# neptune-ai/open-solution-salt-identification

Measured on AMD Instinct MI355X. Metric: training images/sec, U-Net ResNet34 101x101 (pad->128) bs32/GPU, higher is better.
Workload: dtype bf16; 1 GPU; architectures.unet.UNetResNet(34, hypercolumn) 128x128 (101 resized+edge-padded) batch 32/GPU, lovasz loss, Adam lr1e-4 L2 1e-4, train-mode BN; global_batch=32, parallelism=dp1

## Files before the change

include/saltnet.h:

```cpp
#ifndef SALTNET_H
#define SALTNET_H
#include <stdint.h>

#ifdef __cplusplus
extern "C" {
#endif

#define SALT_F32 0
#define SALT_BF16 1

#define SALT_OK 0
#define SALT_E_BADARG -1
#define SALT_E_UNSUPPORTED -2
#define SALT_E_LDS -3

#define SALT_MAX_TAPS 16

typedef struct {
    void* p;
    int B;
    int H;
    int W;
    int C;
    int cs;
// ... 183 lines not shown

typedef struct {
    int dtype;
    const float* w;
    int Cout;
    int Cin;
    int K;
    void* wp;
} salt_pack_stem_weight_args;
int salt_pack_stem_weight(const salt_pack_stem_weight_args*, void* stream);

typedef struct {
    const float* g16;
    int Cout;
    int Cin;
    int K;
    float* grad;
    int accumulate;
} salt_stem_grad_unfold_args;
int salt_stem_grad_unfold(const salt_stem_grad_unfold_args*, void* stream);

typedef struct {
    int dtype;
    salt_view x;
    const float* w;
    const float* bias;
    int Cout;
    float* y_nchw;
    salt_view y;
} salt_head1x1_args;
int salt_head1x1(const salt_head1x1_args*, void* stream);
int salt_head1x1_kernel_id(const salt_head1x1_args*);

typedef struct {
    int dtype;
    salt_view x;
    const float* w;
    int Cout;
    const float* dy_nchw;
    salt_view dx;
    int accumulate;
    float* partials;
    int nparts;
    float* gw;
    float* gb;
} salt_head1x1_bwd_args;
// ... 361 lines not shown
    const float* grad;
    float* exp_avg;
    float* exp_avg_sq;
    int64_t n;
    const float* hyper;
} salt_adam_args;
int salt_adam(const salt_adam_args*, void* stream);

typedef struct {
    float* param;
    const float* grad;
    float* exp_avg;
    float* exp_avg_sq;
    int64_t n;
    const float* hyper;
    const void* jobs;
    const int* job_block0;
    int njobs;
    int pack_blocks;
    const int64_t* rest;
    const int* rest_block0;
    int nrest;
    int rest_blocks;
} salt_adam_pack_args;
int salt_adam_pack(const salt_adam_pack_args*, void* stream);
int salt_pack_job_is_vec(const salt_pack_conv_weight_args*);

typedef struct {
    float* hyper;
    int64_t* step;
} salt_adam_tick_args;
int salt_adam_tick(const salt_adam_tick_args*, void* stream);

typedef struct {
    void* p;
    int64_t bytes;
} salt_zero_args;
int salt_zero(const salt_zero_args*, void* stream);

typedef struct {
    const float* logits;
    int V;
    int B;
    int C;
    int H;
    int W;
// ... 412 lines not shown
```

open-solution-salt-identification_amd/csrc/build.py:

```python
import hashlib
import os
import subprocess
import sys
from concurrent.futures import ThreadPoolExecutor

HERE = os.path.dirname(os.path.abspath(__file__))
PKG = os.path.dirname(HERE)
ROOT = os.path.dirname(PKG)
INC = os.path.join(ROOT, 'include')
OBJ = os.path.join(HERE, '_obj')
LIB = os.path.join(PKG, 'libsaltnet_hip.so')
SOURCES = ['runtime.hip', 'conv_mfma.hip', 'conv_wgrad.hip', 'conv_ws.hip', 'conv_thin.hip', 'conv_wgrad_ls.hip', 'conv_small.hip', 'head_fused.hip', 'elementwise.hip', 'hyper.hip', 'se.hip', 'se_res.hip', 'conv_group.hip', 'dense.hip', 'depth.hip', 'classifier.hip', 'stacking.hip', 'loss.hip', 'input.hip', 'augment.hip']
FLAGS = ['--offload-arch=gfx950', '-O3', '-std=c++17', '-fPIC', '-I' + INC, '-I' + HERE, '-Wno-unused-value']


def _hipcc():
    for c in (os.environ.get('HIPCC'), '/opt/rocm/bin/hipcc', 'hipcc'):
        if c and (os.path.isabs(c) and os.path.exists(c) or not os.path.isabs(c)):
            return c
    raise RuntimeError('hipcc not found')


def _digest(path):
    h = hashlib.sha1()
    for p in [path, os.path.join(HERE, 'common.h'), os.path.join(HERE, 'preprocess_common.h'), os.path.join(INC, 'saltnet.h')]:
        with open(p, 'rb') as f:
            h.update(f.read())
    h.update(' '.join(FLAGS).encode())
    return h.hexdigest()


def _compile(src):
    path = os.path.join(HERE, src)
    obj = os.path.join(OBJ, src.replace('.hip', '.o'))
    stamp = obj + '.sha1'
# ... 35 lines not shown
```

open-solution-salt-identification_amd/csrc/conv_mfma.hip:

```cpp
#include <cstdlib>
#include <type_traits>
#include "common.h"

namespace {

struct ConvKP {
    const void* x; const void* w; void* y;
    const float* bias; const float* scale; const float* shift;
    float* stats; float* stats_cnt;
    int B, H, W, Cin, x_cs;
    int Cout, y_cs, OHf, OWf, OH, OW, out_step, out_oy, out_ox;
    int ntaps; int tap_off[SALT_MAX_TAPS];
    int in_step, pad_mode, min_dy, min_dx;
    int th_log2, tw_log2, nb;
    int gen, tw, th, twth;
    unsigned tw_magic, twth_magic;
    int hh, hw;
    int tiles_y, tiles_x;
    int nchunk, a_bytes;
    int relu, accumulate, stats_part0;
    void* strip; int strip_cs, fold_top, fold_bottom, fold_left, fold_right;
    int nphase, m_tiles_ph; int64_t w_phase_elems;
    int fold_fused, ox_shift;
    unsigned hhw_magic, hw_magic;
// ... 1598 lines not shown
        return;
    }
    for (int e = threadIdx.x; e < PACK_EPB; e += 256) {
        const int64_t i = base + e;
        if (i >= total) break;
        const int kc = (int)(i % KCE);
        int64_t r = i / KCE;
        const int n = (int)(r % N); r /= N;
        const int t = (int)(r % a.ntaps);
        const int ch = (int)(r / a.ntaps) * KCE + kc;
        float v = 0.f;
        if (ch < C && a.tap_kh[t] >= 0) {
            const int d0 = a.transpose ? ch : n, d1 = a.transpose ? n : ch;
            v = a.w[(((int64_t)d0 * a.D1 + d1) * a.KH + a.tap_kh[t]) * a.KW + a.tap_kw[t]];
        }
        Elem<T>::st(out + ((((int64_t)(r / a.ntaps) + a.chunk_off) * a.ntaps + t) * NT_ + n + a.n_off) * KCE + kc, v);
    }
}

struct AdamPackKP {
    float* p; const float* g; float* m; float* v; const float* hyper;
    const salt_pack_conv_weight_args* jobs; const int* job_block0; int njobs, pack_blocks;
    const int64_t* rest; const int* rest_block0; int nrest;
};
constexpr int AP_SEG = 64, AP_SEGF = 288;
__global__ __launch_bounds__(256) void adam_pack_kernel(AdamPackKP k) {
    extern __shared__ __attribute__((aligned(16))) float ap_sm[];
    const float lr = k.hyper[0], b1 = k.hyper[1], b2 = k.hyper[2], eps = k.hyper[3], wd = k.hyper[4], bc1 = k.hyper[5], bc2 = k.hyper[6], gs = k.hyper[7];
    const float step_size = lr / bc1, rs = 1.f / sqrtf(bc2);
    const int tid = threadIdx.x;
    if ((int)blockIdx.x < k.pack_blocks) {
        int lo = 0, hi = k.njobs - 1;
        while (lo < hi) { const int mid = (lo + hi + 1) >> 1; if (k.job_block0[mid] <= (int)blockIdx.x) lo = mid; else hi = mid - 1; }
        const salt_pack_conv_weight_args& a = k.jobs[lo];
        const int N = a.D0, C = a.D1, nseg = N * (C / 32);
        const int seg0 = ((int)blockIdx.x - k.job_block0[lo]) * AP_SEG;
        const int64_t wbase = a.w - k.p;
#pragma unroll 3
        for (int it = 0; it < AP_SEG * AP_SEGF / 4 / 256; ++it) {
            const int f = tid + 256 * it, sl = f / (AP_SEGF / 4), fi = f - sl * (AP_SEGF / 4), seg = seg0 + sl;
            if (seg < nseg) {
                const int chunk = seg / N, n = seg - chunk * N;
                const int64_t off = wbase + ((int64_t)n * C + chunk * 32) * 9 + 4 * fi;
                f32x4 pp = *reinterpret_cast<const f32x4*>(k.p + off);
                const f32x4 gg = *reinterpret_cast<const f32x4*>(k.g + off);
                f32x4 mm = *reinterpret_cast<const f32x4*>(k.m + off), vv = *reinterpret_cast<const f32x4*>(k.v + off);
                adam4(pp, gg, mm, vv, b1, b2, eps, wd, gs, step_size, rs);
                *reinterpret_cast<f32x4*>(k.p + off) = pp; *reinterpret_cast<f32x4*>(k.m + off) = mm; *reinterpret_cast<f32x4*>(k.v + off) = vv;
                *reinterpret_cast<f32x4*>(ap_sm + sl * AP_SEGF + 4 * fi) = pp;
            }
        }
        __syncthreads();
        const int sl = tid >> 2, q = tid & 3, seg = seg0 + sl;
        if (seg >= nseg) return;
        const int chunk = seg / N, n = seg - chunk * N;
        const float* v = ap_sm + sl * AP_SEGF + q * 72;
        bf16_t* out = reinterpret_cast<bf16_t*>(a.wp);
#pragma unroll
        for (int t = 0; t < 9; ++t) {
            u32x4 o;
            o.x = f2bf_pk(v[0 * 9 + t], v[1 * 9 + t]); o.y = f2bf_pk(v[2 * 9 + t], v[3 * 9 + t]);
            o.z = f2bf_pk(v[4 * 9 + t], v[5 * 9 + t]); o.w = f2bf_pk(v[6 * 9 + t], v[7 * 9 + t]);
            *reinterpret_cast<u32x4*>(out + (((int64_t)chunk * 9 + t) * N + n) * 32 + q * 8) = o;
        }
        return;
    }
    const int rb = (int)blockIdx.x - k.pack_blocks;
    int lo = 0, hi = k.nrest - 1;
    while (lo < hi) { const int mid = (lo + hi + 1) >> 1; if (k.rest_block0[mid] <= rb) lo = mid; else hi = mid - 1; }
    const int64_t first = k.rest[2 * lo], count = k.rest[2 * lo + 1];
    const int64_t e = (int64_t)(rb - k.rest_block0[lo]) * 1024 + tid * 4;
    if (e >= count) return;
    const int64_t off = first + e;
    f32x4 pp = *reinterpret_cast<const f32x4*>(k.p + off);
    const f32x4 gg = *reinterpret_cast<const f32x4*>(k.g + off);
    f32x4 mm = *reinterpret_cast<const f32x4*>(k.m + off), vv = *reinterpret_cast<const f32x4*>(k.v + off);
    adam4(pp, gg, mm, vv, b1, b2, eps, wd, gs, step_size, rs);
    *reinterpret_cast<f32x4*>(k.p + off) = pp; *reinterpret_cast<f32x4*>(k.m + off) = mm; *reinterpret_cast<f32x4*>(k.v + off) = vv;
}

}

extern "C" int salt_conv(const salt_conv_args* a, void* stream) {
    Plan pl;
    int rc = make_plan(a, &pl);
    if (rc) return rc;
// ... 75 lines not shown
    if (pack_vec_ok(*a, a->dtype)) return (int)(((int64_t)N * (C / 32) * 4 + 255) / 256);
    if (!a->transpose) return (int)(((int64_t)N * cdiv(C, KCE) * KCE + 255) / 256);
    const int64_t total = (int64_t)cdiv(C, KCE) * a->ntaps * N * KCE;
    return (int)((total + PACK_EPB - 1) / PACK_EPB);
}

extern "C" int salt_pack_job_is_vec(const salt_pack_conv_weight_args* a) {
    return a && !a->transpose && a->KH * a->KW == 9 && pack_vec_ok(*a, a->dtype) ? 1 : 0;
}

extern "C" int salt_adam_pack(const salt_adam_pack_args* a, void* stream) {
    if (!a || !a->param || !a->grad || !a->exp_avg || !a->exp_avg_sq || !a->hyper || a->n < 0 || a->njobs < 0 || a->nrest < 0 || a->pack_blocks < 0 ||
        a->rest_blocks < 0 || (a->njobs && (!a->jobs || !a->job_block0)) || (a->nrest && (!a->rest || !a->rest_block0)))
        SALT_FAIL(SALT_E_BADARG, "adam_pack: bad args");
    if ((reinterpret_cast<uintptr_t>(a->param) | reinterpret_cast<uintptr_t>(a->grad) | reinterpret_cast<uintptr_t>(a->exp_avg) | reinterpret_cast<uintptr_t>(a->exp_avg_sq)) & 15)
        SALT_FAIL(SALT_E_BADARG, "adam_pack: buffers must be 16-byte aligned");
    const int64_t blocks = (int64_t)a->pack_blocks + a->rest_blocks;
    if (blocks == 0) return SALT_OK;
    if (blocks >= (1LL << 31)) SALT_FAIL(SALT_E_UNSUPPORTED, "adam_pack: too many blocks");
    AdamPackKP k;
    k.p = a->param; k.g = a->grad; k.m = a->exp_avg; k.v = a->exp_avg_sq; k.hyper = a->hyper;
    k.jobs = reinterpret_cast<const salt_pack_conv_weight_args*>(a->jobs); k.job_block0 = a->job_block0; k.njobs = a->njobs; k.pack_blocks = a->pack_blocks;
    k.rest = a->rest; k.rest_block0 = a->rest_block0; k.nrest = a->nrest;
    return salt_launch(adam_pack_kernel, dim3((unsigned)blocks), dim3(256), AP_SEG * AP_SEGF * sizeof(float), (hipStream_t)stream, k);
}

extern "C" int salt_pack_batched(const salt_pack_batched_args* a, void* stream) {
    if (!a || !a->jobs || !a->job_block0 || a->njobs < 1 || a->total_blocks < 1) SALT_FAIL(SALT_E_BADARG, "pack_batched: bad args");
    const auto* jobs = reinterpret_cast<const salt_pack_conv_weight_args*>(a->jobs);
    if (a->dtype == SALT_F32) hipLaunchKernelGGL(pack_batched_kernel<float>, dim3(a->total_blocks), dim3(256), 0, (hipStream_t)stream, jobs, a->job_block0, a->njobs);
    else if (a->dtype == SALT_BF16) hipLaunchKernelGGL(pack_batched_kernel<bf16_t>, dim3(a->total_blocks), dim3(256), 0, (hipStream_t)stream, jobs, a->job_block0, a->njobs);
    else SALT_FAIL(SALT_E_BADARG, "pack_batched: dtype");
    SALT_CHECK_LAUNCH();
    return SALT_OK;
}
```

open-solution-salt-identification_amd/csrc/runtime.hip:

```cpp
#include <stdarg.h>
#include <string.h>
#include <stdlib.h>
#include "common.h"

static thread_local char g_err[512] = "";

void salt_set_error(const char* fmt, ...) {
    va_list ap;
    va_start(ap, fmt);
    vsnprintf(g_err, sizeof(g_err), fmt, ap);
    va_end(ap);
}

extern "C" const char* salt_last_error(void) { return g_err; }

extern "C" int salt_abi_version(void) { return 30; }

extern "C" int salt_device_info(int* cu_count, int* lds_bytes, char* arch_name, int arch_name_len) {
    int dev = 0;
    hipError_t e = hipGetDevice(&dev);
    if (e != hipSuccess) SALT_FAIL((int)e, "hipGetDevice: %s", hipGetErrorString(e));
    hipDeviceProp_t prop;
    e = hipGetDeviceProperties(&prop, dev);
    if (e != hipSuccess) SALT_FAIL((int)e, "hipGetDeviceProperties: %s", hipGetErrorString(e));
    if (cu_count) *cu_count = prop.multiProcessorCount;
    if (lds_bytes) *lds_bytes = (int)prop.sharedMemPerBlock;
    if (arch_name && arch_name_len > 0) { strncpy(arch_name, prop.gcnArchName, arch_name_len - 1); arch_name[arch_name_len - 1] = 0; }
    return SALT_OK;
}

extern "C" int salt_program_run_range(const salt_program_entry* e, int begin, int end, void* stream) {
    if (!e || begin < 0 || end < begin) SALT_FAIL(SALT_E_BADARG, "program: bad range");
    for (int i = begin; i < end; ++i) {
        const int rc = e[i].fn(e[i].args, stream);
        if (rc) {
            char prev[400];
            strncpy(prev, g_err, sizeof(prev) - 1); prev[sizeof(prev) - 1] = 0;
            salt_set_error("program entry %d failed (%d): %s", i, rc, prev);
            return rc;
// ... 210 lines not shown
extern "C" int salt_zero(const salt_zero_args* a, void* stream) {
    if (!a || !a->p || a->bytes < 0 || (a->bytes & 3)) SALT_FAIL(SALT_E_BADARG, "zero: bad args");
    if (a->bytes == 0) return SALT_OK;
    const int64_t n4 = a->bytes / 4;
    const int blocks = (int)((n4 + 255) / 256 < 2048 ? (n4 + 255) / 256 : 2048);
    hipLaunchKernelGGL(zero_kernel, dim3(blocks), dim3(256), 0, (hipStream_t)stream, (uint32_t*)a->p, n4);
    SALT_CHECK_LAUNCH();
    return SALT_OK;
}

extern "C" int salt_abi_struct_sizes(int* out, int n) {
    static const int sizes[] = {
    (int)sizeof(salt_view),
    (int)sizeof(salt_conv_args),
    (int)sizeof(salt_conv_wgrad_args),
    (int)sizeof(salt_wgrad_reduce_args),
    (int)sizeof(salt_pack_conv_weight_args),
    (int)sizeof(salt_pack_batched_args),
    (int)sizeof(salt_conv_first_args),
    (int)sizeof(salt_conv_first_wgrad_args),
    (int)sizeof(salt_s2d_args),
    (int)sizeof(salt_pack_stem_weight_args),
    (int)sizeof(salt_stem_grad_unfold_args),
    (int)sizeof(salt_head1x1_args),
    (int)sizeof(salt_head1x1_bwd_args),
    (int)sizeof(salt_bn_finalize_args),
    (int)sizeof(salt_bn_fold_args),
    (int)sizeof(salt_affine_act_args),
    (int)sizeof(salt_bn_bwd_args),
    (int)sizeof(salt_head_bn_args),
    (int)sizeof(salt_head_bn_bwd_args),
    (int)sizeof(salt_relu_bwd_args),
    (int)sizeof(salt_maxpool2_args),
    (int)sizeof(salt_maxpool2_bwd_args),
    (int)sizeof(salt_avgpool2_args),
    (int)sizeof(salt_bilinear_args),
    (int)sizeof(salt_hyper_stencil_args),
    (int)sizeof(salt_pad_fold_args),
    (int)sizeof(salt_pad_fold_strip_args),
    (int)sizeof(salt_add_args),
    (int)sizeof(salt_layout_args),
    (int)sizeof(salt_scse_args),
    (int)sizeof(salt_scse_bwd_args),
    (int)sizeof(salt_depth_gate_args),
    (int)sizeof(salt_channel_gate_args),
    (int)sizeof(salt_lovasz_args),
// ... 32 lines not shown
```

open-solution-salt-identification_amd/engine.py:

```python
import contextlib
import ctypes
from collections import namedtuple
from dataclasses import dataclass, field
from typing import Any

import numpy as np
import torch

from . import switches
from ._abi import OP_FUNCS, STRUCTS, SaltError, check, fill, lib

DT_CODE = {'f32': 0, 'bf16': 1}
TORCH_DT = {'f32': torch.float32, 'bf16': torch.bfloat16}
VEC = {'f32': 4, 'bf16': 8}

PARTIALS_OWN = 0
PARTIALS_FILLED = 1
PARTIALS_FINALIZED = 2
PARTIALS_SHARDS = 3

SUMS_OWN = 'own'
SUMS_CONV = 'conv'
SUMS_SEC = 'sec'
SUMS_SCSE = 'scse'
# ... 1059 lines not shown
            self.tape.append(backward)
        else:
            w = eng.bn_work(bn)
            self.fwd.add('conv_first', y=out.view(), scale=w['scale'].data_ptr(), shift=w['shift'].data_ptr(), relu=int(relu), **common)
        return out

    def _stem_s2d(self, x_nchw, conv, bn, relu, name):
        eng = self.engine
        B, Cin, H, W = x_nchw.shape
        Cout, _, K, _ = conv.weight.shape
        TT, half = (K + 1) // 2, (K + 1) // 4
        z = self.new_act(B, H // 2, W // 2, 16, name + '.s2d')
        self.fwd.add('s2d', dtype=self.dt, x=x_nchw.data_ptr(), B=B, Cin=Cin, H=H, W=W, z=z.view())
        wp = eng.packed_stem(conv)
        taps = [(dh - half, dw - half) for dh in range(TT) for dw in range(TT)]
        OH, OW = H // 2, W // 2
        out = self.new_act(B, OH, OW, Cout, name)
        if self.train:
            y = self.new_act(B, OH, OW, Cout, name + '.y')
            w, _ = self._conv_bn_train(z, y, [(wp.data_ptr(), taps, 1, 0, OH, OW, {})], bn, relu, None, out, self._scratch_sfx)

            def backward():
                self._bn_train_bwd(y, bn, relu, None, out, w)
                g16 = self.f32(Cout * 16 * TT * TT)
                gw_tmp = g16.data_ptr()
                per = 8 if len(taps) > 9 else 9
                for i in range(0, len(taps), per):
                    chunk = list(range(i, min(i + per, len(taps))))
                    wg = dict(dtype=self.dt, ntaps=len(chunk), tap_dy=[taps[j][0] for j in chunk], tap_dx=[taps[j][1] for j in chunk], q_step=1, pad_mode=0)
                    ns = lib.salt_conv_wgrad_nsplit(ctypes.byref(fill(STRUCTS['salt_conv_wgrad_args'](), p=y.gview(), q=z.view(), **wg)))
                    nbytes = ns * len(chunk) * Cout * 16 * 4
                    self.bwd.add('conv_wgrad', stream=0, p=y.gview(), q=z.view(), partials=Scratch('wgrad@main', nbytes), nsplit=ns, **wg)
                    self.bwd.add('wgrad_reduce', stream=0, partials=Scratch('wgrad@main', nbytes), nsplit=ns, ntaps=len(chunk), Ca=Cout, Cb=16, KH=TT, KW=TT,
                                 tap_kh=[j // TT for j in chunk], tap_kw=[j % TT for j in chunk], grad=gw_tmp, accumulate=0)
                self.bwd.add('stem_grad_unfold', stream=0, g16=gw_tmp, Cout=Cout, Cin=Cin, K=K, grad=self._gp(conv.weight), accumulate=0)
            self.tape.append(backward)
        else:
            w = eng.bn_work(bn)
            self._conv_launch(self.fwd, z.view(), wp.data_ptr(), taps, 1, 0, out.view(), OH, OW,
                              scale=w['scale'].data_ptr(), shift=w['shift'].data_ptr(), relu=int(relu))
        return out

    def stack_conv(self, x_nchw, conv, bn, relu=True, head=None, gate=None, logits=None, name='stack'):
        eng = self.engine
        B, M, H, W = x_nchw.shape
        F = conv.weight.shape[0]
# ... 474 lines not shown
```

open-solution-salt-identification_amd/optim.py:

```python

import torch

from ._abi import SaltError
from .engine import Program


def weight_regularization(model, regularize, weight_decay_conv2d):
    params = [p for p in model.parameters() if p.requires_grad]
    if regularize:
        return [{'params': params, 'weight_decay': weight_decay_conv2d}]
    return [params]


class FusedAdam(torch.optim.Optimizer):

    def __init__(self, param_groups, lr=1e-3, betas=(0.9, 0.999), eps=1e-8, weight_decay=0.0, model=None):
        if isinstance(param_groups, (list, tuple)) and param_groups and isinstance(param_groups[0], dict):
            g = dict(param_groups[0])
        else:
            g = {'params': list(param_groups[0] if param_groups and isinstance(param_groups[0], (list, tuple)) else param_groups)}
        super().__init__([g], dict(lr=lr, betas=betas, eps=eps, weight_decay=weight_decay))
        if len(self.param_groups) != 1:
            raise SaltError('FusedAdam: one parameter group (models.py:289-297)')
        self.param_groups[0].setdefault('initial_lr', self.param_groups[0]['lr'])
# ... 5 lines not shown

    def _bind(self):
        eng = self.model.engine()
        if self._eng is eng:
            return
        old = (self.exp_avg, self.exp_avg_sq) if self._eng is not None else None
        self._eng = eng
        dev = eng.device
        if old is not None and old[0].numel() == eng.flat.numel():
            self.exp_avg, self.exp_avg_sq = old[0].to(dev).clone(), old[1].to(dev).clone()
        else:
            if old is not None:
                self.steps = 0
            self.exp_avg = torch.zeros_like(eng.flat)
            self.exp_avg_sq = torch.zeros_like(eng.flat)
        self.hyper = torch.zeros(8, dtype=torch.float32, device=dev)
        self.step_t = torch.full((1,), self.steps, dtype=torch.int64, device=dev)
        self._host_hyper = None
        self.prog = Program('adam')
        self.prog.add('adam_tick', hyper=self.hyper.data_ptr(), step=self.step_t.data_ptr())
        self.prog.add('adam', param=eng.flat.data_ptr(), grad=eng.grads.data_ptr(), exp_avg=self.exp_avg.data_ptr(),
                      exp_avg_sq=self.exp_avg_sq.data_ptr(), n=eng.n_live, hyper=self.hyper.data_ptr())
        self.prog.finalize()
        self._pack_prog, self._pack_gen = None, None

    def _adam_pack_program(self):
        import numpy as np
        eng = self._eng
        if eng.dtype != 'bf16':
            return None
        if eng._pack_batched_n != len(eng._pack_ops):
            eng._build_pack_batch()
            eng._packed_version = eng._packed_bwd_version = -1
        if self._pack_gen == eng._pack_generation:
            return self._pack_prog
        self._pack_gen, self._pack_prog = eng._pack_generation, None
        jobs = eng._adam_jobs
        if not jobs:
            return None
        import ctypes
        from ._abi import lib
        base = eng.flat.data_ptr()
        blocks = [lib.salt_pack_job_blocks(ctypes.byref(j)) for j in jobs]
        pref = np.concatenate([[0], np.cumsum(blocks)]).astype(np.int32)
        covered = sorted(((j.w - base) // 4, j.D0 * j.D1 * j.KH * j.KW) for j in jobs)
        rest, pos = [], 0
        for first, cnt in covered:
            if first % 4 or cnt % 4 or first < pos:
                return None
            if first > pos:
                rest.append((pos, first - pos))
            pos = first + cnt
        if pos < eng.n_live:
            rest.append((pos, eng.n_live - pos))
        rblocks = [(c + 1023) // 1024 for _, c in rest]
        rpref = np.concatenate([[0], np.cumsum(rblocks)]).astype(np.int32) if rest else np.zeros(1, np.int32)
        dev = eng.device
        self._pack_tables = [torch.frombuffer(bytearray(b''.join(bytes(j) for j in jobs)), dtype=torch.uint8).to(dev), torch.from_numpy(pref).to(dev),
                             torch.tensor(rest if rest else [[0, 0]], dtype=torch.int64).to(dev), torch.from_numpy(rpref).to(dev)]
        t = self._pack_tables
        prog = Program('adam_pack')
        prog.add('adam_tick', hyper=self.hyper.data_ptr(), step=self.step_t.data_ptr())
        prog.add('adam_pack', param=eng.flat.data_ptr(), grad=eng.grads.data_ptr(), exp_avg=self.exp_avg.data_ptr(), exp_avg_sq=self.exp_avg_sq.data_ptr(),
                 n=eng.n_live, hyper=self.hyper.data_ptr(), jobs=t[0].data_ptr(), job_block0=t[1].data_ptr(), njobs=len(jobs), pack_blocks=int(pref[-1]),
                 rest=t[2].data_ptr(), rest_block0=t[3].data_ptr(), nrest=len(rest), rest_blocks=int(rpref[-1]))
        prog.finalize()
        self._pack_prog = prog
        return prog

    def _sync_hyper(self):
        g = self.param_groups[0]
        cur = (float(g['lr']), float(g['betas'][0]), float(g['betas'][1]), float(g['eps']), float(g['weight_decay']), float(self.grad_scale))
        if cur != self._host_hyper:
            self.hyper[:5].copy_(torch.tensor(cur[:5], dtype=torch.float32))
            self.hyper[7:8].fill_(cur[5])
            self._host_hyper = cur

    def zero_grad(self, set_to_none=False):
        pass

    def step(self, closure=None):
        if self.model is None:
            raise SaltError('FusedAdam needs the HipNetwork it optimises (model=...)')
        self._bind()
        fused = self._adam_pack_program()
        self._sync_hyper()
        (fused or self.prog).run()
        self.steps += 1
        self._eng.touch(weights=True, stats=False)
        if fused is not None:
            self._eng._adam_packed_version = self._eng.wver

    def state_dict(self):
        g = {k: v for k, v in self.param_groups[0].items() if k != 'params'}
        g['params'] = list(range(len(self.param_groups[0]['params'])))
        st = {}
        if self._eng is None and self.model is not None and getattr(self.model, '_engine', None) is not None:
            self._bind()
        if self._eng is not None:
            st = {'step': self.steps, 'exp_avg': self.exp_avg.detach().cpu(), 'exp_avg_sq': self.exp_avg_sq.detach().cpu()}
        return {'state': st, 'param_groups': [g]}

    def load_state_dict(self, sd):
        for k, v in sd['param_groups'][0].items():
            if k != 'params':
                self.param_groups[0][k] = v
        st = sd.get('state', {})
        if st:
            self._bind()
            self.steps = int(st['step'])
            self.step_t.fill_(self.steps)
            self.exp_avg.copy_(st['exp_avg'])
            self.exp_avg_sq.copy_(st['exp_avg_sq'])
```

open-solution-salt-identification_amd/runtime.py:

```python
import ctypes

import torch

from . import _abi
from ._abi import SaltError, lib
from .engine import Graph, Program, DT_CODE, TORCH_DT


def _require_gpu(device):
    if device.type != 'cuda':
        raise SaltError('the HIP path needs a GPU tensor/device (got %s); there is no CPU fallback' % device)


def _ptr_fields(struct, ptr, out):
    for name, ct in struct._fields_:
        v = getattr(struct, name)
        if isinstance(v, ctypes.Structure):
            _ptr_fields(v, ptr, out)
        elif isinstance(v, ctypes.Array):
            for e in v:
                if isinstance(e, ctypes.Structure):
                    _ptr_fields(e, ptr, out)
        elif ct is ctypes.c_void_p and v == ptr:
            out.append((struct, name))
# ... 103 lines not shown
class Engine:
    def __init__(self, module, device, dtype='f32'):
        _require_gpu(device)
        if dtype not in DT_CODE:
            raise SaltError('dtype must be f32 or bf16')
        self.module, self.device, self.dtype = module, device, dtype
        self._flatten()
        self._packed = {}
        self._pack_ops = Program('pack')
        self._packed_bwd_version = -1
        self._pack_is_bwd, self._pack_keys = {}, []
        self._bn = {}
        self._fold_ops = Program('bn_fold')
        self.nets = {}
        self.wver = 0
        self.sver = 0
        self._packed_version = -1
        self._folded_version = None
        self.world = 1
        self.side_stream = torch.cuda.Stream(device=device)
        self._pack_generation = 0
        self._pack_batched_n = -1
        self._adam_packed_version = None
        self._graph_stream = None
        self._pack_fork = None
        self.eager_done = set()

    def _flatten(self):
        m = self.module
        dead = set(m.dead_parameter_names()) if hasattr(m, 'dead_parameter_names') else set()
        seen = {}
        live = []
        for name, p in m.named_parameters():
            if id(p) in seen:
                continue
            seen[id(p)] = name
            if p.requires_grad and name not in dead:
                live.append((name, p))
        total = sum(((p.numel() + 3) // 4) * 4 for _, p in live)
        self.flat = torch.zeros(total, dtype=torch.float32, device=self.device)
        self.grads = torch.zeros(total, dtype=torch.float32, device=self.device)
        self._off = {}
        self.live_names = []
        off = 0
        for name, p in live:
            n = p.numel()
# ... 140 lines not shown
                pref = np.concatenate([[0], np.cumsum(blocks)]).astype(np.int32)
                table = torch.frombuffer(bytearray(raw), dtype=torch.uint8).to(self.device)
                pref_t = torch.from_numpy(pref).to(self.device)
                self._pack_tables += [table, pref_t]
                prog.add('pack_batched', jobs=table.data_ptr(), job_block0=pref_t.data_ptr(), njobs=len(sel), total_blocks=int(pref[-1]),
                         dtype=DT_CODE[self.dtype])
            return prog
        fwd_jobs = [s for s, k in zip(jobs, self._pack_keys) if not self._pack_is_bwd[k]]
        fwd = batch(fwd_jobs, 'pack')
        fwd.extend(others)
        fwd.finalize()
        lo, hi = self.flat.data_ptr(), self.flat.data_ptr() + 4 * self.n_live
        seen, self._adam_jobs = set(), []
        for s in fwd_jobs:
            if lib.salt_pack_job_is_vec(ctypes.byref(s)) and lo <= s.w < hi and s.w not in seen:
                seen.add(s.w)
                self._adam_jobs.append(s)
        ids = {id(s) for s in self._adam_jobs}
        rest = batch([s for s in fwd_jobs if id(s) not in ids], 'pack_rest')
        rest.extend(others)
        rest.finalize()
        self._pack_batched_rest = rest
        self._adam_packed_version = None
        bwd = batch([s for s, k in zip(jobs, self._pack_keys) if self._pack_is_bwd[k]], 'pack_bwd')
        bwd.finalize()
        self._pack_batched, self._pack_batched_bwd = fwd, bwd
        self._pack_batched_n = len(self._pack_ops)
        self._pack_generation += 1

    def refresh(self, train):
        if self._pack_batched_n != len(self._pack_ops):
            self._build_pack_batch()
            self._packed_version = self._packed_bwd_version = -1
        if self._packed_version != self.wver:
            (self._pack_batched_rest if self._adam_packed_version == self.wver else self._pack_batched).run()
            self._packed_version = self.wver
        if train and self._packed_bwd_version != self.wver and len(self._pack_batched_bwd):
            self.side_stream.wait_stream(torch.cuda.current_stream())
            self._pack_batched_bwd.run(stream=self.side_stream)
            self._packed_bwd_version = self.wver
        if not train and self._folded_version != (self.wver, self.sver):
            self._fold_ops.run()
            self._folded_version = (self.wver, self.sver)

    def net(self, shape, train):
        key = (tuple(shape), bool(train))
        if key not in self.nets:
            self.nets[key] = CompiledNet(self, tuple(shape), train, self.module.num_classes)
        return self.nets[key]

    def step_graph(self, net, kind, loss_scale, optimizer):
        cache = net.__dict__.setdefault('_step_graphs', {})
        key = (kind, float(loss_scale))
        if self._pack_batched_n != len(self._pack_ops):
            self._build_pack_batch()
        hit = cache.get(key)
        if hit is not None and hit[0] is optimizer and hit[2] == self._pack_generation:
            return hit[1]
        if hit is not None:
            lib.salt_graph_destroy(hit[1])
        optimizer._bind()
        optimizer._sync_hyper()
# ... 69 lines not shown
```

open-solution-salt-identification_amd/switches.py:

```python
import os


def _nonempty(raw):
    return bool(raw)


def _not0(raw):
    return raw != '0'


def _on(raw):
    return raw not in ('', '0')


SWITCHES = {
    'SALT_LIB': ('', str, 'path of a libsaltnet_hip.so build variant to load instead of the package\'s own (tools/build_variant.sh)'),
    'SALT_DTYPE': ('f32', str, 'compute dtype of a network that does not name one (f32 | bf16)'),
    'SALT_STEP_GRAPH': (None, lambda raw: bool(int(raw)), '1 / 0: replay the one-GPU training step as a hipGraph; unset: training_config[\'step_graph\']'),
    'SALT_BN_FIN': (2, int, 'how train-mode BatchNorm sums travel: 2 fp64 shard atomics finalized by the consumer, 1 finalized in the producing launch, 0 per-tile partials (fixed summation order)'),
    'SALT_SE_SHARDS': (True, _not0, '0: scSE per-image sums through per-part partials (fixed summation order) instead of the fp64 shards'),
    'SALT_FWD_BN_FOLD': (False, _on, '1: BatchNorm apply + ReLU folded into the consuming convolution\'s loader; such a graph is forward-only'),
    'SALT_NO_PLANAR': (False, _nonempty, 'hypercolumn stored as channel-interleaved rows instead of dense planes'),
    'SALT_NO_SHORTCUT_FIRST': (False, _nonempty, 'projection shortcut emitted after the main branch, as the reference orders it'),
    'SALT_NO_RES_FOLD': (False, _nonempty, 'residual add + ReLU as separate launches instead of the BatchNorm apply\'s epilogue'),
    'SALT_BNB_SEC': (True, _not0, '0: a projection shortcut\'s BatchNorm backward keeps its own reduction pass'),
    'SALT_HEAD_BN': (True, _not0, '0: final BatchNorm apply and 1x1 logit head as separate launches'),
    'SALT_HYPER_FACTOR': (4, int, 'hypercolumn levels up-sampled by at least this factor enter the final convolution factored (0: none)'),
    'SALT_SE_IN_BN': (True, _not0, '0: scSE reads a materialised activation instead of applying BatchNorm + ReLU itself'),
    'SALT_SE_FC_SIDE': (True, _not0, '0: scSE backward\'s FC weight gradients on the main stream'),
    'SALT_SE_BNB': (True, _not0, '0: scSE backward does not carry the BatchNorm-backward sums of its input\'s producer'),
    'SALT_SE_RES_IN_BN': (True, _not0, '0: the SE-ResNet block tail reads the materialised BatchNorm output instead of applying scale / shift itself (measured 0.2 ms per step slower, DESIGN 16; tools/seresnet_bench.py)'),
    'SALT_RCCL_MAX_NCHANNELS': (0, int, '> 0: export NCCL_MAX_NCHANNELS=<n> before the process group is created'),
    'SALT_NO_PIN': (False, _nonempty, 'leave the process\'s CPU affinity alone'),
    'SALT_FORCE_DP_PATH': (False, _nonempty, 'one rank runs the bucketed all-reduce backward (bench.py, tools/dp_overhead.py)'),
}


def get(name):
    try:
        default, parse, _ = SWITCHES[name]
    except KeyError:
        raise KeyError('%s is not a switch of this package (switches.SWITCHES)' % name) from None
    raw = os.environ.get(name)
    return default if raw is None else parse(raw)
```

Measured before the change: 6475 images/s.

## Add dedicated stem weight-gradient kernel and emit transposed backward weights from Adam pack

```diff
diff --git a/include/saltnet.h b/include/saltnet.h
--- a/include/saltnet.h
+++ b/include/saltnet.h
@@ -229,6 +229,25 @@
 
 typedef struct {
     int dtype;
+    salt_view p;
+    salt_view q;
+    float* partials;
+    int nsplit;
+} salt_stem_wgrad_args;
+int salt_stem_wgrad_nsplit(const salt_stem_wgrad_args*);
+int salt_stem_wgrad(const salt_stem_wgrad_args*, void* stream);
+
+typedef struct {
+    const float* partials;
+    int nsplit;
+    int Cin;
+    float* grad;
+    int accumulate;
+} salt_stem_wgrad_reduce_args;
+int salt_stem_wgrad_reduce(const salt_stem_wgrad_reduce_args*, void* stream);
+
+typedef struct {
+    int dtype;
     salt_view x;
     const float* w;
     const float* bias;
@@ -636,6 +655,7 @@
     const int* rest_block0;
     int nrest;
     int rest_blocks;
+    const void* wp_t;
 } salt_adam_pack_args;
 int salt_adam_pack(const salt_adam_pack_args*, void* stream);
 int salt_pack_job_is_vec(const salt_pack_conv_weight_args*);
diff --git a/open-solution-salt-identification_amd/csrc/build.py b/open-solution-salt-identification_amd/csrc/build.py
--- a/open-solution-salt-identification_amd/csrc/build.py
+++ b/open-solution-salt-identification_amd/csrc/build.py
@@ -10,7 +10,7 @@
 INC = os.path.join(ROOT, 'include')
 OBJ = os.path.join(HERE, '_obj')
 LIB = os.path.join(PKG, 'libsaltnet_hip.so')
-SOURCES = ['runtime.hip', 'conv_mfma.hip', 'conv_wgrad.hip', 'conv_ws.hip', 'conv_thin.hip', 'conv_wgrad_ls.hip', 'conv_small.hip', 'head_fused.hip', 'elementwise.hip', 'hyper.hip', 'se.hip', 'se_res.hip', 'conv_group.hip', 'dense.hip', 'depth.hip', 'classifier.hip', 'stacking.hip', 'loss.hip', 'input.hip', 'augment.hip']
+SOURCES = ['runtime.hip', 'conv_mfma.hip', 'conv_wgrad.hip', 'conv_ws.hip', 'conv_thin.hip', 'conv_wgrad_ls.hip', 'conv_small.hip', 'stem_wgrad.hip', 'head_fused.hip', 'elementwise.hip', 'hyper.hip', 'se.hip', 'se_res.hip', 'conv_group.hip', 'dense.hip', 'depth.hip', 'classifier.hip', 'stacking.hip', 'loss.hip', 'input.hip', 'augment.hip']
 FLAGS = ['--offload-arch=gfx950', '-O3', '-std=c++17', '-fPIC', '-I' + INC, '-I' + HERE, '-Wno-unused-value']
 
 
diff --git a/open-solution-salt-identification_amd/csrc/conv_mfma.hip b/open-solution-salt-identification_amd/csrc/conv_mfma.hip
--- a/open-solution-salt-identification_amd/csrc/conv_mfma.hip
+++ b/open-solution-salt-identification_amd/csrc/conv_mfma.hip
@@ -1644,6 +1644,7 @@
     float* p; const float* g; float* m; float* v; const float* hyper;
     const salt_pack_conv_weight_args* jobs; const int* job_block0; int njobs, pack_blocks;
     const int64_t* rest; const int* rest_block0; int nrest;
+    void* const* wp_t;
 };
 constexpr int AP_SEG = 64, AP_SEGF = 288;
 __global__ __launch_bounds__(256) void adam_pack_kernel(AdamPackKP k) {
@@ -1674,16 +1675,31 @@
         }
         __syncthreads();
         const int sl = tid >> 2, q = tid & 3, seg = seg0 + sl;
-        if (seg >= nseg) return;
-        const int chunk = seg / N, n = seg - chunk * N;
-        const float* v = ap_sm + sl * AP_SEGF + q * 72;
-        bf16_t* out = reinterpret_cast<bf16_t*>(a.wp);
-#pragma unroll
-        for (int t = 0; t < 9; ++t) {
+        if (seg < nseg) {
+            const int chunk = seg / N, n = seg - chunk * N;
+            const float* v = ap_sm + sl * AP_SEGF + q * 72;
+            bf16_t* out = reinterpret_cast<bf16_t*>(a.wp);
+#pragma unroll
+            for (int t = 0; t < 9; ++t) {
+                u32x4 o;
+                o.x = f2bf_pk(v[0 * 9 + t], v[1 * 9 + t]); o.y = f2bf_pk(v[2 * 9 + t], v[3 * 9 + t]);
+                o.z = f2bf_pk(v[4 * 9 + t], v[5 * 9 + t]); o.w = f2bf_pk(v[6 * 9 + t], v[7 * 9 + t]);
+                *reinterpret_cast<u32x4*>(out + (((int64_t)chunk * 9 + t) * N + n) * 32 + q * 8) = o;
+            }
+        }
+        bf16_t* out_t = k.wp_t ? reinterpret_cast<bf16_t*>(k.wp_t[lo]) : nullptr;
+        if (!out_t) return;
+#pragma unroll
+        for (int it = 0; it < 9; ++it) {
+            const int pi = tid + 256 * it, h = pi / 1152, r = pi - h * 1152;
+            const int t = r >> 7, ci = (r >> 2) & 31, qt = r & 3, segh = seg0 + 32 * h;
+            if (segh >= nseg) continue;
+            const int chunk = segh / N, n0 = segh - chunk * N;
+            const float* v = ap_sm + (32 * h + qt * 8) * AP_SEGF + ci * 9 + t;
             u32x4 o;
-            o.x = f2bf_pk(v[0 * 9 + t], v[1 * 9 + t]); o.y = f2bf_pk(v[2 * 9 + t], v[3 * 9 + t]);
-            o.z = f2bf_pk(v[4 * 9 + t], v[5 * 9 + t]); o.w = f2bf_pk(v[6 * 9 + t], v[7 * 9 + t]);
-            *reinterpret_cast<u32x4*>(out + (((int64_t)chunk * 9 + t) * N + n) * 32 + q * 8) = o;
+            o.x = f2bf_pk(v[0], v[AP_SEGF]); o.y = f2bf_pk(v[2 * AP_SEGF], v[3 * AP_SEGF]);
+            o.z = f2bf_pk(v[4 * AP_SEGF], v[5 * AP_SEGF]); o.w = f2bf_pk(v[6 * AP_SEGF], v[7 * AP_SEGF]);
+            *reinterpret_cast<u32x4*>(out_t + (((int64_t)(n0 >> 5) * 9 + t) * C + chunk * 32 + ci) * 32 + qt * 8) = o;
         }
         return;
     }
@@ -1805,6 +1821,7 @@
     k.p = a->param; k.g = a->grad; k.m = a->exp_avg; k.v = a->exp_avg_sq; k.hyper = a->hyper;
     k.jobs = reinterpret_cast<const salt_pack_conv_weight_args*>(a->jobs); k.job_block0 = a->job_block0; k.njobs = a->njobs; k.pack_blocks = a->pack_blocks;
     k.rest = a->rest; k.rest_block0 = a->rest_block0; k.nrest = a->nrest;
+    k.wp_t = reinterpret_cast<void* const*>(a->wp_t);
     return salt_launch(adam_pack_kernel, dim3((unsigned)blocks), dim3(256), AP_SEG * AP_SEGF * sizeof(float), (hipStream_t)stream, k);
 }
 
diff --git a/open-solution-salt-identification_amd/csrc/runtime.hip b/open-solution-salt-identification_amd/csrc/runtime.hip
--- a/open-solution-salt-identification_amd/csrc/runtime.hip
+++ b/open-solution-salt-identification_amd/csrc/runtime.hip
@@ -14,7 +14,7 @@
 
 extern "C" const char* salt_last_error(void) { return g_err; }
 
-extern "C" int salt_abi_version(void) { return 30; }
+extern "C" int salt_abi_version(void) { return 31; }
 
 extern "C" int salt_device_info(int* cu_count, int* lds_bytes, char* arch_name, int arch_name_len) {
     int dev = 0;
@@ -271,6 +271,8 @@
     (int)sizeof(salt_s2d_args),
     (int)sizeof(salt_pack_stem_weight_args),
     (int)sizeof(salt_stem_grad_unfold_args),
+    (int)sizeof(salt_stem_wgrad_args),
+    (int)sizeof(salt_stem_wgrad_reduce_args),
     (int)sizeof(salt_head1x1_args),
     (int)sizeof(salt_head1x1_bwd_args),
     (int)sizeof(salt_bn_finalize_args),
diff --git a/open-solution-salt-identification_amd/csrc/stem_wgrad.hip b/open-solution-salt-identification_amd/csrc/stem_wgrad.hip
--- /dev/null
+++ b/open-solution-salt-identification_amd/csrc/stem_wgrad.hip
@@ -0,0 +1,165 @@
+#include "common.h"
+
+namespace {
+
+constexpr int SW_TW = 16, SW_TH = 8, SW_PIX = SW_TW * SW_TH;
+constexpr int SW_HW = SW_TW + 3, SW_HH = SW_TH + 3;
+constexpr int SW_PROWB = 192, SW_QROWB = 32;
+constexpr int SW_NP = SW_PIX * 8 / 256;
+constexpr int SW_QPIECES = SW_HW * SW_HH * 2, SW_NQ = (SW_QPIECES + 255) / 256;
+constexpr int SW_SLAB = 64 * 256;
+constexpr int SW_MAX_SPLIT = 256;
+constexpr int SW_RG = 16;
+
+struct StemWgradKP {
+    const bf16_t* P; const bf16_t* Q; float* partials;
+    int B, OH, OW, p_cs, q_cs;
+    int tiles_y, tiles_x, ntiles, nsplit;
+};
+
+__global__ __launch_bounds__(256) void stem_wgrad_kernel(StemWgradKP p) {
+    typedef short s16x4 __attribute__((ext_vector_type(4)));
+    typedef short s16x8 __attribute__((ext_vector_type(8)));
+    typedef __attribute__((address_space(3))) s16x4* lds_s16x4_ptr;
+    __shared__ __attribute__((aligned(16))) unsigned char sP[SW_PIX * SW_PROWB];
+    __shared__ __attribute__((aligned(16))) unsigned char sQ[SW_HW * SW_HH * SW_QROWB];
+    const int tid = threadIdx.x, lane = tid & 63, wave = tid >> 6;
+    const int split = blockIdx.x;
+
+    f32x16 acc[2][2];
+#pragma unroll
+    for (int i = 0; i < 4; ++i)
+#pragma unroll
+        for (int r = 0; r < 16; ++r) acc[i >> 1][i & 1][r] = 0.f;
+
+    int p_ty[SW_NP], p_tx[SW_NP], q_hy[SW_NQ], q_hx[SW_NQ];
+#pragma unroll
+    for (int k = 0; k < SW_NP; ++k) { const int m = (tid + (k << 8)) >> 3; p_ty[k] = m >> 4; p_tx[k] = m & 15; }
+#pragma unroll
+    for (int k = 0; k < SW_NQ; ++k) { const int hp = (tid + (k << 8)) >> 1; q_hy[k] = hp / SW_HW; q_hx[k] = hp - q_hy[k] * SW_HW; }
+    const int p_ch = (tid & 7) * 8, q_ch = (tid & 1) * 8;
+    u32x4 rp[SW_NP], rq[SW_NQ];
+    auto load_tile = [&](int tile) {
+        const int txi = tile % p.tiles_x, tt = tile / p.tiles_x, tyi = tt % p.tiles_y, b = tt / p.tiles_y;
+        const int y0 = tyi * SW_TH, x0 = txi * SW_TW;
+        const bf16_t* Pb = p.P + (int64_t)b * p.OH * p.OW * p.p_cs;
+        const bf16_t* Qb = p.Q + (int64_t)b * p.OH * p.OW * p.q_cs;
+#pragma unroll
+        for (int k = 0; k < SW_NP; ++k) {
+            const int oy = y0 + p_ty[k], ox = x0 + p_tx[k];
+            rp[k] = u32x4{0u, 0u, 0u, 0u};
+            if (oy < p.OH && ox < p.OW) rp[k] = *reinterpret_cast<const u32x4*>(Pb + (oy * p.OW + ox) * p.p_cs + p_ch);
+        }
+#pragma unroll
+        for (int k = 0; k < SW_NQ; ++k) {
+            const int iy = y0 + q_hy[k] - 2, ix = x0 + q_hx[k] - 2;
+            rq[k] = u32x4{0u, 0u, 0u, 0u};
+            if (tid + (k << 8) < SW_QPIECES && (unsigned)iy < (unsigned)p.OH && (unsigned)ix < (unsigned)p.OW)
+                rq[k] = *reinterpret_cast<const u32x4*>(Qb + (iy * p.OW + ix) * p.q_cs + q_ch);
+        }
+    };
+
+    const int khalf = lane >> 5, g16 = (lane >> 4) & 1, i16 = lane & 15, prow = i16 >> 2, pcol = (i16 & 3) * 4;
+    const int pa_base = (khalf * 8 + prow) * SW_PROWB + (g16 * 16 + pcol) * 2;
+    const int qa_base = (wave * SW_HW + khalf * 8 + prow + g16) * SW_QROWB + pcol * 2;
+
+    if (split < p.ntiles) load_tile(split);
+    for (int tile = split; tile < p.ntiles; tile += p.nsplit) {
+        __syncthreads();
+#pragma unroll
+        for (int k = 0; k < SW_NP; ++k) { const int q = tid + (k << 8); *reinterpret_cast<u32x4*>(sP + (q >> 3) * SW_PROWB + (q & 7) * 16) = rp[k]; }
+#pragma unroll
+        for (int k = 0; k < SW_NQ; ++k) { const int q = tid + (k << 8); if (q < SW_QPIECES) *reinterpret_cast<u32x4*>(sQ + q * 16) = rq[k]; }
+        __syncthreads();
+        if (tile + p.nsplit < p.ntiles) load_tile(tile + p.nsplit);
+#pragma unroll
+        for (int j = 0; j < SW_TH; ++j) {
+            s16x4 fa[2][2], fb[2][2];
+#pragma unroll
+            for (int i = 0; i < 2; ++i)
+#pragma unroll
+                for (int h = 0; h < 2; ++h) {
+                    fa[i][h] = __builtin_amdgcn_ds_read_tr16_b64_v4i16((lds_s16x4_ptr)(sP + pa_base + (j * SW_TW + 4 * h) * SW_PROWB + i * 64));
+                    fb[i][h] = __builtin_amdgcn_ds_read_tr16_b64_v4i16((lds_s16x4_ptr)(sQ + qa_base + (j * SW_HW + 4 * h + 2 * i) * SW_QROWB));
+                }
+#pragma unroll
+            for (int at = 0; at < 2; ++at) {
+                const s16x8 av = {fa[at][0][0], fa[at][0][1], fa[at][0][2], fa[at][0][3], fa[at][1][0], fa[at][1][1], fa[at][1][2], fa[at][1][3]};
+#pragma unroll
+                for (int nt = 0; nt < 2; ++nt) {
+                    const s16x8 bv = {fb[nt][0][0], fb[nt][0][1], fb[nt][0][2], fb[nt][0][3], fb[nt][1][0], fb[nt][1][1], fb[nt][1][2], fb[nt][1][3]};
+                    acc[at][nt] = __builtin_amdgcn_mfma_f32_32x32x16_bf16(__builtin_bit_cast(bf16x8, bv), __builtin_bit_cast(bf16x8, av), acc[at][nt], 0, 0, 0);
+                }
+            }
+        }
+    }
+    float* slab = p.partials + (int64_t)split * SW_SLAB;
+#pragma unroll
+    for (int at = 0; at < 2; ++at)
+#pragma unroll
+        for (int nt = 0; nt < 2; ++nt)
+#pragma unroll
+            for (int g = 0; g < 4; ++g) {
+                const int a = at * 32 + (lane & 31);
+                const int n = (wave * 4 + nt * 2) * 16 + 8 * g + 4 * khalf;
+                const f32x16& v = acc[at][nt];
+                *reinterpret_cast<f32x4*>(slab + ((n >> 2) * 64 + a) * 4) = f32x4{v[4 * g], v[4 * g + 1], v[4 * g + 2], v[4 * g + 3]};
+            }
+}
+
+__global__ __launch_bounds__(64 * SW_RG) void stem_wgrad_reduce_kernel(const float* partials, int nsplit, int Cin, float* grad, int accumulate) {
+    __shared__ float red[SW_RG][64];
+    const int j = threadIdx.x & 63, r = threadIdx.x >> 6;
+    const int e = blockIdx.x * 64 + j;
+    const int per = (nsplit + SW_RG - 1) / SW_RG;
+    const int s0 = r * per, s1 = min(s0 + per, nsplit);
+    float v = 0.f;
+#pragma unroll 8
+    for (int s = s0; s < s1; ++s) v += partials[(int64_t)s * SW_SLAB + e];
+    red[r][j] = v;
+    __syncthreads();
+    if (r) return;
+#pragma unroll
+    for (int q = 1; q < SW_RG; ++q) v += red[q][j];
+    const int a = (e >> 2) & 63, n = ((e >> 8) << 2) | (e & 3), t = n >> 4, c16 = n & 15;
+    if (c16 >= 4 * Cin) return;
+    const int pp = c16 / Cin, c = c16 - pp * Cin;
+    const int kh = 2 * ((t >> 2) - 2) + (pp >> 1) + 3, kw = 2 * ((t & 3) - 2) + (pp & 1) + 3;
+    if (kh < 0 || kw < 0) return;
+    float* d = grad + ((a * Cin + c) * 7 + kh) * 7 + kw;
+    *d = accumulate ? *d + v : v;
+}
+
+bool stem_wgrad_plan(const salt_stem_wgrad_args* a, StemWgradKP* kp) {
+    if (!a || a->dtype != SALT_BF16 || !view_ok(a->p) || !view_ok(a->q)) return false;
+    if (a->p.C != 64 || a->q.C != 16 || a->p.B != a->q.B || a->p.H != a->q.H || a->p.W != a->q.W) return false;
+    if ((a->p.cs & 7) || (a->q.cs & 7) || (reinterpret_cast<uintptr_t>(a->p.p) & 15) || (reinterpret_cast<uintptr_t>(a->q.p) & 15)) return false;
+    if ((int64_t)a->p.H * a->p.W * a->p.cs >= (1ll << 31)) return false;
+    const int64_t ntiles = (int64_t)a->p.B * cdiv(a->p.H, SW_TH) * cdiv(a->p.W, SW_TW);
+    if (ntiles >= (1ll << 31)) return false;
+    kp->P = (const bf16_t*)a->p.p; kp->Q = (const bf16_t*)a->q.p; kp->partials = a->partials;
+    kp->B = a->p.B; kp->OH = a->p.H; kp->OW = a->p.W; kp->p_cs = a->p.cs; kp->q_cs = a->q.cs;
+    kp->tiles_y = cdiv(a->p.H, SW_TH); kp->tiles_x = cdiv(a->p.W, SW_TW); kp->ntiles = (int)ntiles;
+    kp->nsplit = kp->ntiles < SW_MAX_SPLIT ? kp->ntiles : SW_MAX_SPLIT;
+    return true;
+}
+
+}
+
+extern "C" int salt_stem_wgrad_nsplit(const salt_stem_wgrad_args* a) {
+    StemWgradKP kp;
+    if (!stem_wgrad_plan(a, &kp)) SALT_FAIL(SALT_E_BADARG, "stem_wgrad: bf16 dL/dy [B,H,W,64] and z [B,H,W,16] with 16-byte aligned pixels expected");
+    return kp.nsplit;
+}
+
+extern "C" int salt_stem_wgrad(const salt_stem_wgrad_args* a, void* stream) {
+    StemWgradKP kp;
+    if (!stem_wgrad_plan(a, &kp) || !a->partials) SALT_FAIL(SALT_E_BADARG, "stem_wgrad: bf16 dL/dy [B,H,W,64], z [B,H,W,16] with 16-byte aligned pixels and a workspace expected");
+    if (a->nsplit != kp.nsplit) SALT_FAIL(SALT_E_BADARG, "stem_wgrad: nsplit %d, the plan has %d (salt_stem_wgrad_nsplit)", a->nsplit, kp.nsplit);
+    return salt_launch(stem_wgrad_kernel, dim3(kp.nsplit), dim3(256), 0, (hipStream_t)stream, kp);
+}
+
+extern "C" int salt_stem_wgrad_reduce(const salt_stem_wgrad_reduce_args* a, void* stream) {
+    if (!a || !a->partials || !a->grad || a->nsplit < 1 || a->Cin < 1 || a->Cin > 4) SALT_FAIL(SALT_E_BADARG, "stem_wgrad_reduce: bad args");
+    return salt_launch(stem_wgrad_reduce_kernel, dim3(SW_SLAB / 64), dim3(64 * SW_RG), 0, (hipStream_t)stream, a->partials, a->nsplit, a->Cin, a->grad, a->accumulate);
+}
diff --git a/open-solution-salt-identification_amd/engine.py b/open-solution-salt-identification_amd/engine.py
--- a/open-solution-salt-identification_amd/engine.py
+++ b/open-solution-salt-identification_amd/engine.py
@@ -1105,6 +1105,15 @@
 
             def backward():
                 self._bn_train_bwd(y, bn, relu, None, out, w)
+                if self.dt == DT_CODE['bf16'] and K == 7 and Cout == 64 and Cin <= 4 and switches.get('SALT_STEM_WGRAD'):
+                    sw = dict(dtype=self.dt, p=y.gview(), q=z.view())
+                    ns = lib.salt_stem_wgrad_nsplit(ctypes.byref(fill(STRUCTS['salt_stem_wgrad_args'](), **sw)))
+                    if ns < 1:
+                        raise SaltError('stem: weight-gradient plan failed: ' + lib.salt_last_error().decode())
+                    slabs = Scratch('wgrad@main', ns * 64 * 256 * 4)
+                    self.bwd.add('stem_wgrad', stream=0, partials=slabs, nsplit=ns, **sw)
+                    self.bwd.add('stem_wgrad_reduce', stream=0, partials=slabs, nsplit=ns, Cin=Cin, grad=self._gp(conv.weight), accumulate=0)
+                    return
                 g16 = self.f32(Cout * 16 * TT * TT)
                 gw_tmp = g16.data_ptr()
                 per = 8 if len(taps) > 9 else 9
diff --git a/open-solution-salt-identification_amd/optim.py b/open-solution-salt-identification_amd/optim.py
--- a/open-solution-salt-identification_amd/optim.py
+++ b/open-solution-salt-identification_amd/optim.py
@@ -51,7 +51,7 @@
         self.prog.add('adam', param=eng.flat.data_ptr(), grad=eng.grads.data_ptr(), exp_avg=self.exp_avg.data_ptr(),
                       exp_avg_sq=self.exp_avg_sq.data_ptr(), n=eng.n_live, hyper=self.hyper.data_ptr())
         self.prog.finalize()
-        self._pack_prog, self._pack_gen = None, None
+        self._pack_prog, self._pack_gen, self._packs_bwd = None, None, False
 
     def _adam_pack_program(self):
         import numpy as np
@@ -87,12 +87,17 @@
         dev = eng.device
         self._pack_tables = [torch.frombuffer(bytearray(b''.join(bytes(j) for j in jobs)), dtype=torch.uint8).to(dev), torch.from_numpy(pref).to(dev),
                              torch.tensor(rest if rest else [[0, 0]], dtype=torch.int64).to(dev), torch.from_numpy(rpref).to(dev)]
+        twins = [(t.wp if t is not None else 0) for t in eng._adam_jobs_t]
+        self._packs_bwd = any(twins)
+        if self._packs_bwd:
+            self._pack_tables.append(torch.tensor(twins, dtype=torch.int64).to(dev))
         t = self._pack_tables
         prog = Program('adam_pack')
         prog.add('adam_tick', hyper=self.hyper.data_ptr(), step=self.step_t.data_ptr())
         prog.add('adam_pack', param=eng.flat.data_ptr(), grad=eng.grads.data_ptr(), exp_avg=self.exp_avg.data_ptr(), exp_avg_sq=self.exp_avg_sq.data_ptr(),
                  n=eng.n_live, hyper=self.hyper.data_ptr(), jobs=t[0].data_ptr(), job_block0=t[1].data_ptr(), njobs=len(jobs), pack_blocks=int(pref[-1]),
-                 rest=t[2].data_ptr(), rest_block0=t[3].data_ptr(), nrest=len(rest), rest_blocks=int(rpref[-1]))
+                 rest=t[2].data_ptr(), rest_block0=t[3].data_ptr(), nrest=len(rest), rest_blocks=int(rpref[-1]),
+                 wp_t=t[4].data_ptr() if self._packs_bwd else None)
         prog.finalize()
         self._pack_prog = prog
         return prog
@@ -119,6 +124,8 @@
         self._eng.touch(weights=True, stats=False)
         if fused is not None:
             self._eng._adam_packed_version = self._eng.wver
+            if self._packs_bwd:
+                self._eng._adam_packed_bwd_version = self._eng.wver
 
     def state_dict(self):
         g = {k: v for k, v in self.param_groups[0].items() if k != 'params'}
diff --git a/open-solution-salt-identification_amd/runtime.py b/open-solution-salt-identification_amd/runtime.py
--- a/open-solution-salt-identification_amd/runtime.py
+++ b/open-solution-salt-identification_amd/runtime.py
@@ -149,6 +149,7 @@
         self._pack_generation = 0
         self._pack_batched_n = -1
         self._adam_packed_version = None
+        self._adam_packed_bwd_version = None
         self._graph_stream = None
         self._pack_fork = None
         self.eager_done = set()
@@ -335,8 +336,21 @@
         rest.finalize()
         self._pack_batched_rest = rest
         self._adam_packed_version = None
-        bwd = batch([s for s, k in zip(jobs, self._pack_keys) if self._pack_is_bwd[k]], 'pack_bwd')
+        bwd_jobs = [s for s, k in zip(jobs, self._pack_keys) if self._pack_is_bwd[k]]
+        bwd = batch(bwd_jobs, 'pack_bwd')
         bwd.finalize()
+        twins = {}
+        for s in bwd_jobs:
+            if (s.transpose == 1 and s.KH * s.KW == 9 and s.ntaps == 9 and s.D0 % 32 == 0 and s.D1 % 32 == 0 and s.wp % 16 == 0
+                    and not (s.d1_cnt or s.n_off or s.n_total or s.chunk_off) and all(s.tap_kh[t] * s.KW + s.tap_kw[t] == t for t in range(9))):
+                twins.setdefault(s.w, s)
+        self._adam_jobs_t = [twins.get(s.w) for s in self._adam_jobs]
+        self._adam_jobs_t = [t if t is not None and (t.D0, t.D1) == (s.D0, s.D1) else None for s, t in zip(self._adam_jobs, self._adam_jobs_t)]
+        tids = {id(t) for t in self._adam_jobs_t if t is not None}
+        bwd_rest = batch([s for s in bwd_jobs if id(s) not in tids], 'pack_bwd_rest')
+        bwd_rest.finalize()
+        self._pack_batched_bwd_rest = bwd_rest
+        self._adam_packed_bwd_version = None
         self._pack_batched, self._pack_batched_bwd = fwd, bwd
         self._pack_batched_n = len(self._pack_ops)
         self._pack_generation += 1
@@ -350,7 +364,9 @@
             self._packed_version = self.wver
         if train and self._packed_bwd_version != self.wver and len(self._pack_batched_bwd):
             self.side_stream.wait_stream(torch.cuda.current_stream())
-            self._pack_batched_bwd.run(stream=self.side_stream)
+            rest = self._pack_batched_bwd_rest if self._adam_packed_bwd_version == self.wver else self._pack_batched_bwd
+            if len(rest):
+                rest.run(stream=self.side_stream)
             self._packed_bwd_version = self.wver
         if not train and self._folded_version != (self.wver, self.sver):
             self._fold_ops.run()
diff --git a/open-solution-salt-identification_amd/switches.py b/open-solution-salt-identification_amd/switches.py
--- a/open-solution-salt-identification_amd/switches.py
+++ b/open-solution-salt-identification_amd/switches.py
@@ -30,6 +30,7 @@
     'SALT_SE_FC_SIDE': (True, _not0, '0: scSE backward\'s FC weight gradients on the main stream'),
     'SALT_SE_BNB': (True, _not0, '0: scSE backward does not carry the BatchNorm-backward sums of its input\'s producer'),
     'SALT_SE_RES_IN_BN': (True, _not0, '0: the SE-ResNet block tail reads the materialised BatchNorm output instead of applying scale / shift itself (measured 0.2 ms per step slower, DESIGN 16; tools/seresnet_bench.py)'),
+    'SALT_STEM_WGRAD': (True, _not0, '0: the bf16 stem\'s weight gradient as two 8-tap launches of the generic kernel, two slab reductions and the unfold instead of salt_stem_wgrad + salt_stem_wgrad_reduce'),
     'SALT_RCCL_MAX_NCHANNELS': (0, int, '> 0: export NCCL_MAX_NCHANNELS=<n> before the process group is created'),
     'SALT_NO_PIN': (False, _nonempty, 'leave the process\'s CPU affinity alone'),
     'SALT_FORCE_DP_PATH': (False, _nonempty, 'one rank runs the bucketed all-reduce backward (bench.py, tools/dp_overhead.py)'),
```

After: 6513 images/s (median of 6 runs). About the same (+0.6%).
